# zhen8838/K210_Yolo_framework

Measured on AMD Instinct MI355X. Metric: images/sec end-to-end, yolo_mobilev1-0.75 320x240 b32 (`value_from_host`: SURVEY 8(d) end to end - u8 frames in pinned host memory -> H2D -> normalise -> backbone + heads -> decode -> NMS -> detections in host memory; `value`: the same step with the frames already resident in HBM, which is what the , higher is better.
Workload: dtype f16x2 (compensated fp16 MFMA operands: x = hi + lo, fp32 accumulate)

## Files before the change

### k210_yolo_framework_amd/csrc/yk_exact.hip

```cpp
#include <algorithm>
#include <math.h>
#include <string>
#include <vector>

#include "yk_conv.h"
#include "yk_plan_graph.h"

namespace {

typedef __attribute__((address_space(3))) void *lds_ptr_t;
typedef uint32_t u32x4 __attribute__((ext_vector_type(4)));
typedef uint32_t u32x2 __attribute__((ext_vector_type(2)));
#define X_OOB 0x40000000u
#ifdef YK_DEV
#define X_DBG(a, bit) (((a).dbg & (bit)) != 0)
#else
#define X_DBG(a, bit) false
#endif

extern __shared__ __attribute__((aligned(16))) unsigned char xsm[];

__device__ __forceinline__ float x_actf(float v, float slope, float cap) { return __builtin_amdgcn_fmed3f(v, v * slope, cap); }
__device__ __forceinline__ uint32_t x_div(uint32_t n, yk_fastdiv d) { return (__umulhi(n, d.mul) + n) >> d.shift; }

// ... 825 lines not shown
    x_amax_lds(&smax, 0, mx);
    __syncthreads();
    if (tid == 0 && smax) x_amax_global(a.amax_out + (size_t)b * XS, smax);
}

enum { XK_STEM = 1, XK_CONV, XK_DW, XK_POOL, XK_ADD, XK_U8MAX, XK_BLOCK, XK_PERSIST, XK_HEADS, XK_FIN };
enum { XC_64x64 = 0, XC_64x128, XC_128x64, XC_128x128, XC_NUM };
struct xc_info {
    int bm, bn, threads;
    const char *name;
};
const xc_info g_xc[XC_NUM] = {{64, 64, 256, "64x64"}, {64, 128, 256, "64x128"}, {128, 64, 256, "128x64"}, {128, 128, 512, "128x128"}};

struct xtens : yk_gtens {
    uint8_t *d = nullptr;
    bool f32 = false;
    float *d32 = nullptr;
};
struct xlaunch {
    int kind = 0;
    xg_args c;
    xdw_args d;
    xstem_args s;
    xpool_args p;
    xadd_args ad;
    xb_args b;
    int tm = 0, tn = 0;
    int Ho = 0, Wo = 0;
    int cfg = 0, ns = 2;
    unsigned lds = 0;
    int in_tid = -1, out_tid = -1;
    unsigned ring_lds = 0;
    xp_args pa;
    xh_args ha;
    unsigned h_lds = 0;
    xf_args f;
    int fin_bn = 0;
    int p_cw = 0;
    std::string name;
    double flops = 0, bytes = 0;
};

template <int BM, int BN, int WM, int WN, int NS>
int x_launch_g(const xg_args &g, hipStream_t st) {
    typedef xg_cfg<BM, BN, WM, WN> C;
    constexpr unsigned lds = (unsigned)C::lds(NS), rlds = (unsigned)(C::CT + C::SMALL);
    dim3 grid((unsigned)((g.M + BM - 1) / BM), (unsigned)((g.N + BN - 1) / BN), (unsigned)g.splitk);
    yk_launch_lds(g.splitk > 1 ? xg_kernel<BM, BN, WM, WN, NS, true> : xg_kernel<BM, BN, WM, WN, NS, false>, grid, dim3(C::NT), lds, st, g);
    if (g.splitk > 1) yk_launch_lds(xg_reduce_kernel<BM, BN, WM, WN>, dim3(grid.x, grid.y), dim3(C::NT), rlds, st, g);
    return YK_OK;
}
template <int BM, int BN, int WM, int WN>
int x_launch_g_ns(const xg_args &g, int ns, hipStream_t st) {
    if (ns <= 2) return x_launch_g<BM, BN, WM, WN, 2>(g, st);
    if (ns == 3) return x_launch_g<BM, BN, WM, WN, 3>(g, st);
    return x_launch_g<BM, BN, WM, WN, 4>(g, st);
}
int x_launch_conv(int cfg, int ns, const xg_args &g, hipStream_t st) {
    switch (cfg) {
    case XC_64x64: return x_launch_g_ns<64, 64, 2, 2>(g, ns, st);
    case XC_64x128: return x_launch_g_ns<64, 128, 2, 2>(g, ns, st);
    case XC_128x64: return x_launch_g_ns<128, 64, 2, 2>(g, ns, st);
    case XC_128x128: return x_launch_g_ns<128, 128, 2, 4>(g, std::min(ns, 3), st);
    }
    yk_set_error("f16x2: bad tile configuration %d", cfg);
    return YK_ERR_ARG;
}

template <int BM, int BN, int NW>
int x_launch_fin_bn(const xf_args &f, int ns, hipStream_t st) {
    typedef xf_cfg<BM, BN, NW> C;
    const dim3 grid((unsigned)((f.c.M + BM - 1) / BM), 1u, (unsigned)f.c.splitk);
    if (ns < 3) yk_launch_lds(xf_kernel<BM, BN, 2, NW>, grid, dim3(C::NT), C::lds(2), st, f);
    else yk_launch_lds(xf_kernel<BM, BN, 3, NW>, grid, dim3(C::NT), C::lds(3), st, f);
    return YK_OK;
}
int x_launch_fin(int bn, int ns, const xf_args &f, hipStream_t st) {
    if (bn == 128) return x_launch_fin_bn<64, 128, 4>(f, ns, st);
    if (bn == 192) return x_launch_fin_bn<64, 192, 4>(f, ns, st);
    yk_set_error("f16x2: no fused head kernel for a 64 x %d tile on 4 waves", bn);
    return YK_ERR_ARG;
}

template <int TM, int TN, int SG, bool F32IN = false>
int x_launch_b2(const xb_args &g, int batch, unsigned lds, hipStream_t st) {
    if constexpr (SG > 0 && !F32IN)
        if (g.in_f32) return x_launch_b2<TM, TN, SG, true>(g, batch, lds, st);
    dim3 grid((unsigned)(batch * g.tiles_x * g.tiles_y), (unsigned)((g.N + 64 * TN - 1) / (64 * TN)));
    yk_launch_lds(xb_kernel<TM, TN, SG, F32IN>, grid, dim3(256), lds, st, g);
    return YK_OK;
}
template <int TM, int TN>
int x_launch_b(const xb_args &g, int batch, unsigned lds, hipStream_t st) {
    if constexpr (TN == 1) {
        if (g.stem && g.GL == 2) return x_launch_b2<TM, TN, 2>(g, batch, lds, st);
        if (g.stem && g.GL == 3) return x_launch_b2<TM, TN, 3>(g, batch, lds, st);
        if (g.stem && g.GL == 4) return x_launch_b2<TM, TN, 4>(g, batch, lds, st);
    }
    if (g.stem) {
        yk_set_error("f16x2: stem fusion needs an N tile of 64 and 16, 24 or 32 stem filters");
        return YK_ERR_UNSUPPORTED;
    }
    return x_launch_b2<TM, TN, 0>(g, batch, lds, st);
}
const int g_xb_tm[] = {2, 3, 4, 5, 8}, g_xb_tn[] = {1, 2, 3, 6};
bool xb_has(int tm, int tn) {
    if (tm * tn > 24) return false;
    bool a = false, b = false;
    for (int v : g_xb_tm) a |= v == tm;
    for (int v : g_xb_tn) b |= v == tn;
    return a && b;
}
int x_launch_block(int tm, int tn, const xb_args &g, int batch, unsigned lds, hipStream_t st) {
#define XB_CASE(M, N) \
    if (tm == M && tn == N) return x_launch_b<M, N>(g, batch, lds, st);
    XB_CASE(2, 1) XB_CASE(2, 2) XB_CASE(2, 3) XB_CASE(2, 6)
    XB_CASE(3, 1) XB_CASE(3, 2) XB_CASE(3, 3) XB_CASE(3, 6)
    XB_CASE(4, 1) XB_CASE(4, 2) XB_CASE(4, 3) XB_CASE(4, 6)
    XB_CASE(5, 1) XB_CASE(5, 2) XB_CASE(5, 3)
    XB_CASE(8, 1) XB_CASE(8, 2) XB_CASE(8, 3)
#undef XB_CASE
    yk_set_error("f16x2: no fused block kernel <%d,%d>", tm, tn);
    return YK_ERR_ARG;
}
int xb_bt_bytes(int tn, int N) { return std::min(64 * tn, (N + 15) / 16 * 16) * 128; }
unsigned xb_lds(int tm, int tn, int n16p, int db, int N, bool wt = false, bool staged = true) {
    const int bm = 16 * tm, bn = 64 * tn;
    const int ipp = (tn >= 3 && tm >= 2) ? (tm + 1) / 2 : tm;
    const int ring = (db ? 2 : 1) * (n16p * 32 + 2048 + (wt ? xb_bt_bytes(tn, N) : 0)) + bm * 128, ct = staged ? ipp * 16 * (bn * 4 + 16) : 0;
    return (unsigned)(std::max(ring, ct) + 64);
}
bool xb_geometry(xb_args &g, int *tm_out, int *tn_out, unsigned *lds_out, int max_batch, int ordinal) {
    const int s = g.stride;
    double best = -1.0;
    const bool mine = !yk_dev_env("YK_XB_LAYER") || atoi(yk_dev_env("YK_XB_LAYER")) == ordinal;
    const int force_tm = mine && yk_dev_env("YK_XB_TM") ? atoi(yk_dev_env("YK_XB_TM")) : 0, force_tn = mine && yk_dev_env("YK_XB_TN") ? atoi(yk_dev_env("YK_XB_TN")) : 0;
    const int force_tw = mine && yk_dev_env("YK_XB_TW") ? atoi(yk_dev_env("YK_XB_TW")) : 0;
    const int force_db = mine && yk_dev_env("YK_XB_DB") ? atoi(yk_dev_env("YK_XB_DB")) : -1;
    const bool forced = force_tm || force_tn || force_tw || force_db >= 0;
    const bool wide = g.N > 192 && g.nk > 6;
    const int tn_want = (wide && yk_dev_env("YK_XB_TNL")) ? atoi(yk_dev_env("YK_XB_TNL")) : (wide ? 6 : std::min(3, (g.N + 63) / 64));
    (void)max_batch;
    for (int tm : g_xb_tm)
        for (int tn : g_xb_tn) {
            if (!xb_has(tm, tn) || (force_tm && tm != force_tm) || (force_tn && tn != force_tn)) continue;
            if (!force_tn && tn != tn_want) continue;
            const int tm_long = yk_dev_env("YK_XB_TML") ? atoi(yk_dev_env("YK_XB_TML")) : 4;
            if (!force_tm && tm > (tn_want == 1 ? 8 : (g.nk > 6 ? tm_long : 4))) continue;
            const int bm = 16 * tm;
            for (int TW = 1; TW <= std::min(g.Wo, bm); ++TW) {
                if (force_tw && TW != force_tw) continue;
                const int TH = std::min(g.Ho, bm / TW);
                if (TH * TW <= 16 * (tm - 1)) continue;
                const int PH = (TH - 1) * s + 3, PW = (TW - 1) * s + 3;
                const int n16 = PH * PW * 4, n16p = (n16 + 63) & ~63;
                if (n16p > 1536) continue;
                for (int db = 0; db <= 1; ++db) {
                    if (force_db >= 0 ? db != force_db : db != 0) continue;
                    const unsigned lds = xb_lds(tm, tn, n16p, db, g.N);
                    if (lds > 160 * 1024 || (!forced && xb_lds(tm, tn, n16p, db, g.N, !wide) > 53 * 1024 + 512)) continue;
                    const long tiles = (long)((g.Ho + TH - 1) / TH) * ((g.Wo + TW - 1) / TW);
                    const double cover = (double)g.Ho * g.Wo / ((double)tiles * bm);
                    const double halo = (double)TH * TW * s * s / ((double)PH * PW);
                    const double score = bm * cover * (0.5 + 0.5 * halo) * (TW >= TH ? 1.0 : 0.999) * ((TW & 3) ? 0.98 : 1.0);
                    if (score > best) {
                        best = score;
                        *tm_out = tm; *tn_out = tn; *lds_out = lds;
                        g.TH = TH; g.TW = TW; g.PH = PH; g.PW = PW; g.n16 = n16; g.n16p = n16p; g.db = db;
                        g.lds_bytes = (int)lds;
                        g.prepass = (s == 1 && yk_dev_env("YK_XB_PREPASS")) ? 1 : 0;
                        g.tiles_x = (g.Wo + TW - 1) / TW;
                        g.tiles_y = (g.Ho + TH - 1) / TH;
                    }
                }
            }
        }
    if (best < 0) return false;
    g.fd_tpi = yk_make_fastdiv((uint32_t)(g.tiles_x * g.tiles_y));
    g.fd_tx = yk_make_fastdiv((uint32_t)g.tiles_x);
    g.fd_tw = yk_make_fastdiv((uint32_t)g.TW);
    g.fd_pw = yk_make_fastdiv((uint32_t)g.PW);
    g.fd_nk = yk_make_fastdiv((uint32_t)std::max(1, g.nk));
    g.GL = 4;
    return true;
}

}

struct yk_xplan {
    int max_batch = 0, in_h = 0, in_w = 0;
    std::vector<xtens> T;
    std::vector<xlaunch> L;
    yk_dev_mem mem;
    std::vector<int> outputs;
    unsigned *d_imgmax = nullptr;
    uint32_t *d_amax = nullptr;
    size_t zero_words = 0;
    uint32_t *d_err = nullptr;
    uint32_t *h_err = nullptr;
    int *d_eexp = nullptr;
    long long *d_dbg = nullptr;
    int dbg_launch = -1;
    int cluster_wt = 0;
};

void yk_xplan_destroy(yk_xplan *p) {
    if (!p) return;
    p->mem.free_all();
    if (p->h_err) (void)hipHostFree(p->h_err);
    delete p;
}


static int x_build_persist(yk_xplan *p, int max_batch) {
    constexpr int CW = 8;
    const unsigned ring_cap = XP_NS * 8 * 6 * 1024;
    auto pw_ok = [&](const xlaunch &l) {
        const xg_args &g = l.c;
        return l.kind == XK_CONV && g.ks == 1 && g.stride == 1 && !g.s1.p && !g.up0 && !g.res.p && g.splitk == 1 && g.out && l.in_tid >= 0 &&
               (g.N % (16 * CW)) == 0 && (g.s0.G % CW) == 0 && (g.s0.G % 4) == 0;
    };
    auto dw_ok = [&](const xlaunch &l) { return l.kind == XK_DW && (l.d.in.G % CW) == 0 && (l.d.in.G % 4) == 0; };
    auto y_fits = [&](int H, int W, int Gs) { return (unsigned)(2 * (H + 2) * (W + 2) * Gs * 16) <= ring_cap; };
    int best0 = -1, best1 = -1;
    const int n = (int)p->L.size();
    for (int i = 0; i < n; ++i) {
        if (!dw_ok(p->L[i])) continue;
        int k = i, blocks = 0;
        while (k + 1 < n && dw_ok(p->L[k]) && pw_ok(p->L[k + 1]) && p->L[k + 1].in_tid == p->L[k].out_tid && p->T[p->L[k].out_tid].uses == 1) {
            const xdw_args &d = p->L[k].d;
            const xg_args &g = p->L[k + 1].c;
            const int nrb = (d.Ho * d.Wo + 15) / 16, ncb = g.N / 16 / CW, nT = 2 * (nrb + ncb);
            bool ok = nT <= 48 && y_fits(d.in.H, d.in.W, d.in.G / CW) && y_fits(d.Ho, d.Wo, g.N / 8 / CW) && d.in.H * d.in.W <= 1024;
            bool tile = false;
            for (int wr = 8; wr >= 1 && !tile; wr >>= 1) tile = (nrb + wr - 1) / wr <= 3 && (ncb + 8 / wr - 1) / (8 / wr) <= 3;
            if (!ok || !tile) break;
            ++blocks;
            k += 2;
            if (!(k < n && dw_ok(p->L[k]) && p->L[k].in_tid == p->L[k - 1].out_tid)) break;
        }
        if (blocks >= 2 && blocks * 2 > best1 - best0 + 1) {
            best0 = i;
            best1 = i + 2 * blocks - 1;
        }
        if (blocks) i = i + 2 * blocks - 1;
    }
    if (best0 < 0) return YK_OK;
    std::vector<xp_phase> ph;
    std::vector<std::pair<uint32_t, const xlaunch *>> wcopy;
    uint32_t arena = 0, dmax = 0;
    double flops = 0, bytes = 0;
    int nbar = 0, dbuf = 0;
    auto zero_phase = [] {
        xp_phase q;
        memset(&q, 0, sizeof(q));
        return q;
    };
    for (int k = best0; k <= best1; k += 2) {
        const xlaunch &ld = p->L[k], &lp = p->L[k + 1];
        const xdw_args &d = ld.d;
        const xg_args &g = lp.c;
        flops += ld.flops + lp.flops;
        bytes += ld.bytes + lp.bytes;
        const int Gs_in = d.in.G / CW, Gs_out = g.N / 8 / CW;
        if (k == best0) {
            xp_phase q = zero_phase();
// ... 475 lines not shown
```

### k210_yolo_framework_amd/csrc/yk_xblock.h

```cpp
#pragma once

struct xb_args {
    xview in, res;
    int B, Ho, Wo, N;
    int stride, pad_t, pad_l;
    const float *par;
    int nk;
    float dw_slope, dw_cap, dw_gain, dw_off;
    const uint8_t *w;
    uint32_t w_bytes;
    int nslab;
    const float *scale, *bias;
    float slope, cap, gain, off;
    uint8_t *out;
    int outG;
    int *eexp_out;
    uint32_t *amax_out;
    int TH, TW, PH, PW, tiles_x, tiles_y, n16, n16p;
    int db;
    int prepass;
    int src_f32, dst_f32;
    int lds_bytes;
    yk_fastdiv fd_tpi, fd_tx, fd_tw, fd_pw, fd_nk;
    int stem;
    const void *frames;
    const unsigned *img_max;
    int in_f32, fH, fW;
    int st_stride, st_pad_t, st_pad_l, st_cout;
    const yk_half *st_wf;
    const float *st_scale, *st_bias;
    float st_slope, st_cap, st_bound;
    int st_e;
    yk_fastdiv fd_wrow;
    yk_fastdiv fd_dpr;
    int GL;
    int dbg;
    long long *stamps;
};

template <int TM, int TN>
struct xb_cfg {
    static constexpr int BM = 16 * TM, BN = 64 * TN;
    static constexpr int PARB = 2048;
    static constexpr int CPITCH = BN * 4 + 16;
    static constexpr int IPP = (TN >= 3 && TM >= 2) ? (TM + 1) / 2 : TM;
    static constexpr int stage(int n16p) { return n16p * 32 + PARB; }
    static constexpr int lds(int n16p, int db) {
        const int r = (db ? 2 : 1) * stage(n16p) + BM * 128, ct = IPP * 16 * CPITCH;
        return (r > ct ? r : ct) + 64;
    }
};

template <bool U8, int GL>
__device__ __forceinline__ void xb_stem_patch(const xb_args &a, const void *winp, int WC, int pitch, float inv, int iy0, int ix0, unsigned char *HI, unsigned char *LO) {
    const int lane = threadIdx.x & 63, wid = threadIdx.x >> 6, fr = lane & 15, fq = lane >> 4;
    half8 wfh[2], wfl[2];
    float scv[2][4], bsv[2][4];
    const float sdown = x_pow2(-a.st_e), sfac = U8 ? sdown / inv : sdown, cap = a.st_cap * sdown;
#pragma unroll
    for (int nf = 0; nf < 2; ++nf) {
        wfh[nf] = *reinterpret_cast<const half8 *>(a.st_wf + ((size_t)(nf * 2 + 0) * 64 + lane) * 8);
        wfl[nf] = *reinterpret_cast<const half8 *>(a.st_wf + ((size_t)(nf * 2 + 1) * 64 + lane) * 8);
        const float4 sc = *reinterpret_cast<const float4 *>(a.st_scale + nf * 16 + fq * 4);
        const float4 bs = *reinterpret_cast<const float4 *>(a.st_bias + nf * 16 + fq * 4);
        scv[nf][0] = sc.x * sfac, scv[nf][1] = sc.y * sfac, scv[nf][2] = sc.z * sfac, scv[nf][3] = sc.w * sfac;
        bsv[nf][0] = bs.x * sdown, bsv[nf][1] = bs.y * sdown, bsv[nf][2] = bs.z * sdown, bsv[nf][3] = bs.w * sdown;
    }
    const int st = a.st_stride, npos = a.PH * a.PW, nblk = (npos + 15) >> 4, rowf = WC * 3;
    for (int blk = wid; blk < nblk; blk += 4) {
        const int pos = blk * 16 + fr, pc = min(pos, npos - 1);
        const int r = (int)x_div((uint32_t)pc, a.fd_pw), c = pc - r * a.PW;
        const bool valid = pos < npos;
        const bool inside = valid && (unsigned)(iy0 + r) < (unsigned)a.in.H && (unsigned)(ix0 + c) < (unsigned)a.in.W;
        half8 xh, xl;
        if constexpr (U8) {
            const unsigned char *wb = reinterpret_cast<const unsigned char *>(winp);
            const int off = (r * st) * pitch + c * st * 3;
            uint32_t d0, d1 = 0u;
            if (fq < 3) {
                const int o = off + fq * pitch, sh = o & 3;
                const uint32_t *q = reinterpret_cast<const uint32_t *>(wb + (o & ~3));
                const uint32_t w0 = q[0], w1 = q[1], w2 = q[2];
                d0 = __builtin_amdgcn_alignbyte(w1, w0, sh);
                d1 = __builtin_amdgcn_alignbyte(w2, w1, sh);
            } else {
                d0 = (uint32_t)wb[off + 8] | ((uint32_t)wb[off + pitch + 8] << 8) | ((uint32_t)wb[off + 2 * pitch + 8] << 16);
            }
#pragma unroll
            for (int j = 0; j < 4; ++j) {
                xh[j] = (yk_half)(float)((d0 >> (8 * j)) & 255u);
                xh[4 + j] = (yk_half)(float)((d1 >> (8 * j)) & 255u);
            }
        } else {
            const float *base = reinterpret_cast<const float *>(winp) + ((r * st) * WC + c * st) * 3;
            float x[8];
            if (fq < 3) {
#pragma unroll
                for (int j = 0; j < 8; ++j) x[j] = base[fq * rowf + j];
            } else {
                x[0] = base[8];
                x[1] = base[rowf + 8];
                x[2] = base[2 * rowf + 8];
#pragma unroll
                for (int j = 3; j < 8; ++j) x[j] = 0.f;
            }
            x_split8(x, xh, xl);
        }
        floatx4 acc[2];
#pragma unroll
        for (int nf = 0; nf < 2; ++nf) acc[nf] = __builtin_amdgcn_mfma_f32_16x16x32_f16(wfl[nf], xh, floatx4{0.f, 0.f, 0.f, 0.f}, 0, 0, 0);
        if constexpr (!U8) {
#pragma unroll
            for (int nf = 0; nf < 2; ++nf) acc[nf] = __builtin_amdgcn_mfma_f32_16x16x32_f16(wfh[nf], xl, acc[nf], 0, 0, 0);
        }
#pragma unroll
        for (int nf = 0; nf < 2; ++nf) acc[nf] = __builtin_amdgcn_mfma_f32_16x16x32_f16(wfh[nf], xh, acc[nf], 0, 0, 0);
#pragma unroll
        for (int nf = 0; nf < 2; ++nf) {
            float v[4];
#pragma unroll
            for (int k = 0; k < 4; ++k) {
                const float u = __builtin_fmaf(acc[nf][k], scv[nf][k], bsv[nf][k]);
                v[k] = inside ? x_actf(u, a.st_slope, cap) : 0.f;
            }
            const int n = nf * 16 + fq * 4;
            if (valid && (n >> 3) < GL) {
                const int at = (pos * GL + (n >> 3)) * 16;
                *reinterpret_cast<u32x4 *>(((n & 4) ? LO : HI) + at) = u32x4{__float_as_uint(v[0]), __float_as_uint(v[1]), __float_as_uint(v[2]), __float_as_uint(v[3])};
            }
        }
    }
}

template <int TM, int TN, int SG, bool F32IN = false>
__global__ void __launch_bounds__(256, (TM * TN > 8 ? 2 : 4)) xb_kernel(const xb_args a) {
    typedef xb_cfg<TM, TN> C;
    constexpr int BM = C::BM, BN = C::BN;
    constexpr bool STEM = SG > 0;
    constexpr int GL = STEM ? SG : 4;
    const int tid = threadIdx.x, lane = tid & 63, wid = tid >> 6;
    const int G = a.in.G, s = a.stride;
#ifdef YK_DEV
    const int XB_DB = a.db, XB_PREPASS = a.prepass;
#else
    constexpr int XB_DB = 0, XB_PREPASS = 0;
#endif
#ifdef YK_DEV
#define XB_STAMP(k) \
    if (a.stamps && tid == 0) a.stamps[((size_t)blockIdx.y * gridDim.x + blockIdx.x) * 16 + (k)] = (long long)wall_clock64();
#else
#define XB_STAMP(k)
#endif
    XB_STAMP(0)
    const int STG = a.n16p * 32 + C::PARB;
    unsigned char *A = xsm + (XB_DB ? 2 : 1) * STG;
    float *sf = reinterpret_cast<float *>(xsm + a.lds_bytes - 64);
    uint32_t *smax = reinterpret_cast<uint32_t *>(sf + 8);
    const int bid = x_xcd_tile(blockIdx.x, gridDim.x);
    const uint32_t b = x_div((uint32_t)bid, a.fd_tpi), tl = bid - b * (a.tiles_x * a.tiles_y);
    const uint32_t ty = x_div(tl, a.fd_tx), tx = tl - ty * a.tiles_x;
    const int oy0 = (int)ty * a.TH, ox0 = (int)tx * a.TW;
    const int iy0 = oy0 * s - a.pad_t, ix0 = ox0 * s - a.pad_l;
    const int n0 = blockIdx.y * BN;
    const int fr = lane & 15, fq = lane >> 4, nl4 = fq * 4;
    constexpr bool EARLY_SB = TN <= 1;
    float4 sc[TN], bs[TN];
    if constexpr (EARLY_SB) {
#pragma unroll
        for (int j = 0; j < TN; ++j) {
            const int n = n0 + (wid * TN + j) * 16 + nl4;
            sc[j] = *reinterpret_cast<const float4 *>(a.scale + n);
            bs[j] = *reinterpret_cast<const float4 *>(a.bias + n);
        }
    }
    const uint32_t img = (uint32_t)a.in.H * a.in.W * G * 32u;
    const __amdgpu_buffer_rsrc_t rsx = __builtin_amdgcn_make_buffer_rsrc((void *)(STEM ? (const uint8_t *)a.par : a.in.p + (size_t)b * img), 0, STEM ? 16u : img, 0x00020000);
    const __amdgpu_buffer_rsrc_t rsp = __builtin_amdgcn_make_buffer_rsrc((void *)a.par, 0, (uint32_t)(11 * G * 32), 0x00020000);
    const __amdgpu_buffer_rsrc_t rsw = __builtin_amdgcn_make_buffer_rsrc((void *)a.w, 0, a.w_bytes, 0x00020000);
    constexpr int PQ = 6;
    uint32_t poff[PQ];
#pragma unroll
    for (int i = 0; i < PQ; ++i) {
        poff[i] = X_OOB;
        if (!STEM && i * 256 < a.n16p) {
            const uint32_t q = (uint32_t)(i * 256 + tid);
            const uint32_t pos = q >> 2, g4 = q & 3;
            const uint32_t r = x_div(pos, a.fd_pw), c = pos - r * a.PW;
            const int iy = iy0 + (int)r, ix = ix0 + (int)c;
            const bool ok = (int)q < a.n16 && (unsigned)iy < (unsigned)a.in.H && (unsigned)ix < (unsigned)a.in.W;
            poff[i] = ok ? (uint32_t)(((iy * a.in.W + ix) * G + (int)g4) * 32) : X_OOB;
        }
    }
    const int g4l = tid & 3;
    const int rot = (a.nk == 1 || X_DBG(a, 32)) ? 0 : (int)(tl - x_div(tl, a.fd_nk) * (uint32_t)a.nk);
    auto kstep = [&](int i) {
        const int k = i + rot;
        return k >= a.nk ? k - a.nk : k;
    };
    const uint32_t wstep = (uint32_t)a.nslab * 2048u;
    auto dma_patch = [&](int it_) {
        const int ks = kstep(it_);
        unsigned char *HI = xsm + ((XB_DB & it_) & 1) * STG, *LO = HI + a.n16p * 16, *PARb = HI + a.n16p * 32;
        const bool gok = (ks * 4 + g4l) < G;
        const uint32_t koff = gok ? (uint32_t)ks * 128u : X_OOB;
#pragma unroll
        for (int i = 0; i < PQ; ++i)
            if (!STEM && i * 256 + wid * 64 < a.n16p) {
                const uint32_t oh = poff[i] + koff, ol = oh + 16u;
                __builtin_amdgcn_raw_ptr_buffer_load_lds(rsx, (lds_ptr_t)(HI + (i * 256 + wid * 64) * 16), 16, oh, 0, 0, 0);
                __builtin_amdgcn_raw_ptr_buffer_load_lds(rsx, (lds_ptr_t)(LO + (i * 256 + wid * 64) * 16), 16, ol, 0, 0, 0);
            }
        if (wid < 2) {
            const int idx = wid * 64 + lane, t = idx >> 3, pc = idx & 7;
            const int ch = ks * 32 + pc * 4;
            const uint32_t op = (idx < 88 && ch < G * 8) ? (uint32_t)((t * G * 8 + ch) * 4) : X_OOB;
            __builtin_amdgcn_raw_ptr_buffer_load_lds(rsp, (lds_ptr_t)(PARb + wid * 1024), 16, op, 0, 0, 0);
        }
    };
    if (!X_DBG(a, 1)) dma_patch(0);
    if constexpr (STEM) {
        const int st = a.st_stride, WR = (a.PH - 1) * st + 3, WC = (a.PW - 1) * st + 3;
        const int wy0 = iy0 * st - a.st_pad_t, wx0 = ix0 * st - a.st_pad_l;
        float *win = reinterpret_cast<float *>(A);
        float inv = 1.f;
        if (!F32IN) {
            unsigned mx = 0;
#pragma unroll
            for (int j = 0; j < 32; ++j) mx = max(mx, a.img_max[b * 32 + j]);
            inv = (float)mx;
        }
        const int rowf_ = WC * 3;
        if constexpr (F32IN) {
            constexpr int WQ = 16;
            const float *f = reinterpret_cast<const float *>(a.frames);
            const size_t fimg = (size_t)b * a.fH * a.fW * 3;
            float wv[WQ];
            bool wok[WQ];
#pragma unroll
            for (int q = 0; q < WQ; ++q) {
                const int i = q * 256 + tid;
                const int r = (int)x_div((uint32_t)i, a.fd_wrow), rem = i - r * rowf_, c = rem / 3, ch = rem - c * 3;
                const int fy = wy0 + r, fx = wx0 + c;
                wok[q] = i < WR * rowf_ && (unsigned)fy < (unsigned)a.fH && (unsigned)fx < (unsigned)a.fW;
                wv[q] = f[wok[q] ? fimg + ((size_t)fy * a.fW + fx) * 3 + ch : fimg];
            }
#pragma unroll
            for (int q = 0; q < WQ; ++q) {
                const int i = q * 256 + tid;
                if (i < WR * rowf_) win[i] = wok[q] ? wv[q] : 0.f;
            }
        } else {
            constexpr int DQ = 5;
            const int dpr = (rowf_ + 3) >> 2;
            const uint32_t fbytes = (uint32_t)a.B * a.fH * a.fW * 3u;
            const __amdgpu_buffer_rsrc_t rsf = __builtin_amdgcn_make_buffer_rsrc((void *)a.frames, 0, fbytes, 0x00020000);
            const int rowb = a.fW * 3;
            u32x2 d2[DQ];
            int sh[DQ];
            uint32_t msk[DQ];
#pragma unroll
            for (int q = 0; q < DQ; ++q) {
                const int i = q * 256 + tid, r = (int)x_div((uint32_t)i, a.fd_dpr), d = i - r * dpr;
                const int fy = wy0 + r;
                const bool ok = r < WR && (unsigned)fy < (unsigned)a.fH;
                const int col = wx0 * 3 + d * 4;
                const int off = ((int)b * a.fH + fy) * rowb + col;
                sh[q] = off >= 0 ? (off & 3) * 8 : off * 8;
                d2[q] = __builtin_bit_cast(u32x2, __builtin_amdgcn_raw_buffer_load_b64(rsf, ok ? (uint32_t)(max(off, 0) & ~3) : X_OOB, 0, 0));
                const int lo = max(0, -col), hi = min(4, rowb - col);
                msk[q] = (ok && hi > lo) ? ((0xffffffffu << (8 * lo)) & (0xffffffffu >> (8 * (4 - hi)))) : 0u;
            }
#pragma unroll
            for (int q = 0; q < DQ; ++q) {
                const int i = q * 256 + tid;
                const unsigned long long v = ((unsigned long long)d2[q][1] << 32) | d2[q][0];
                const uint32_t dv = sh[q] >= 0 ? (uint32_t)(v >> sh[q]) : (uint32_t)(v << (-sh[q]));
                if (i < WR * dpr) reinterpret_cast<uint32_t *>(A)[i] = dv & msk[q];
            }
            if (tid < 2) reinterpret_cast<uint32_t *>(A)[WR * dpr + tid] = 0u;
        }
        XB_STAMP(11)
        __syncthreads();
        XB_STAMP(12)
        unsigned char *HI = xsm, *LO = xsm + a.n16p * 16;
        if constexpr (F32IN) xb_stem_patch<false, GL>(a, A, WC, 0, 1.f, iy0, ix0, HI, LO);
        else xb_stem_patch<true, GL>(a, A, WC, ((WC * 3 + 3) >> 2) * 4, inv, iy0, ix0, HI, LO);
    }
    XB_STAMP(1)
    if (wid == 0) {
        const float amax_in = STEM ? a.st_bound : x_amax_wave(a.in.amax, (int)b);
        const float bmid = fminf(a.dw_cap, a.dw_gain * amax_in + a.dw_off);
        float bout = fminf(a.cap, a.gain * bmid + a.off);
        float rup = 0.f;
        if (a.res.p) {
            bout += x_amax_wave(a.res.amax, (int)b);
            rup = x_pow2(a.res.eexp[b]);
        }
        const int em = x_exp_of(__float_as_uint(bmid)), eo = a.dst_f32 ? 0 : x_exp_of(__float_as_uint(bout));
        if (lane == 0) {
            sf[0] = x_pow2(STEM ? a.st_e : a.in.eexp[b]);
            sf[1] = x_pow2(-em);
            sf[2] = x_pow2(em);
            sf[3] = x_pow2(-eo);
            sf[4] = rup;
            smax[0] = 0u;
            a.eexp_out[b] = eo;
        }
    }
    XB_STAMP(2)
    floatx4 acc[TM][TN];
#pragma unroll
    for (int i = 0; i < TM; ++i)
#pragma unroll
        for (int j = 0; j < TN; ++j) acc[i][j] = floatx4{0.f, 0.f, 0.f, 0.f};
    const bool wave_live = n0 + wid * TN * 16 < a.N;
    const int foff = fr * 64 + ((fq ^ ((fr >> 1) & 3)) * 16);
    const int afoff = fr * (GL * 16) + (GL == 4 ? (fq ^ ((fr >> 1) & 3)) : (fq < GL ? fq : 0)) * 16;
    const int nk = X_DBG(a, 1) ? 0 : a.nk;
    for (int ks = 0; ks < nk; ++ks) {
        asm volatile("s_waitcnt vmcnt(0) lgkmcnt(0)" ::: "memory");
        __builtin_amdgcn_s_barrier();
        asm volatile("" ::: "memory");
        if (ks == 0) { XB_STAMP(3) }
        if (ks == 1) { XB_STAMP(13) }
        half8 wh[TN], wl[TN];
        if (wave_live && !X_DBG(a, 16)) {
            const uint32_t ws = (uint32_t)(n0 >> 4) * 2048u + (uint32_t)kstep(ks) * wstep + (uint32_t)(wid * TN) * 2048u + (uint32_t)foff;
#pragma unroll
            for (int j = 0; j < TN; ++j) {
                wh[j] = __builtin_bit_cast(half8, __builtin_amdgcn_raw_buffer_load_b128(rsw, ws + (uint32_t)j * 2048u, 0, 0));
                wl[j] = __builtin_bit_cast(half8, __builtin_amdgcn_raw_buffer_load_b128(rsw, ws + (uint32_t)j * 2048u + 1024u, 0, 0));
            }
        }
        if (XB_DB && ks + 1 < nk) dma_patch(ks + 1);
        const unsigned char *HI = xsm + ((XB_DB & ks) & 1) * STG, *LO = HI + a.n16p * 16;
        const unsigned char *PARB_ = HI + a.n16p * 32;
        const float up = sf[0], dmid = sf[1];
        const bool f32patch = STEM || XB_PREPASS || a.src_f32;
        if (!STEM && XB_PREPASS && !a.src_f32) {
            for (int e = tid; e < a.n16p; e += 256) {
                const u32x4 h = *reinterpret_cast<const u32x4 *>(HI + e * 16), l = *reinterpret_cast<const u32x4 *>(LO + e * 16);
                u32x4 x0, x1;
                x0[0] = __float_as_uint(x_mix_sum_lo(h[0], l[0])); x0[1] = __float_as_uint(x_mix_sum_hi(h[0], l[0]));
                x0[2] = __float_as_uint(x_mix_sum_lo(h[1], l[1])); x0[3] = __float_as_uint(x_mix_sum_hi(h[1], l[1]));
                x1[0] = __float_as_uint(x_mix_sum_lo(h[2], l[2])); x1[1] = __float_as_uint(x_mix_sum_hi(h[2], l[2]));
                x1[2] = __float_as_uint(x_mix_sum_lo(h[3], l[3])); x1[3] = __float_as_uint(x_mix_sum_hi(h[3], l[3]));
                *reinterpret_cast<u32x4 *>(const_cast<unsigned char *>(HI) + e * 16) = x0;
                *reinterpret_cast<u32x4 *>(const_cast<unsigned char *>(LO) + e * 16) = x1;
            }
            asm volatile("s_waitcnt lgkmcnt(0)" ::: "memory");
            __builtin_amdgcn_s_barrier();
            asm volatile("" ::: "memory");
        }
        if (!X_DBG(a, 2))
            for (int it = tid; it < BM * GL; it += 256) {
                int p, q;
                if constexpr (GL != 4) {
                    p = (int)((uint32_t)it / (uint32_t)GL);
                    q = it - p * GL;
                } else {
                    p = it >> 2;
                    q = it & 3;
                }
                const int py = (int)x_div((uint32_t)p, a.fd_tw), px = p - py * a.TW;
                const bool live = py < a.TH && oy0 + py < a.Ho && ox0 + px < a.Wo;
                half8 hi = {0, 0, 0, 0, 0, 0, 0, 0}, lo = hi;
                if (live) {
                    const int base = ((py * s) * a.PW + px * s) * GL + q;
                    float2v d2[4] = {{0.f, 0.f}, {0.f, 0.f}, {0.f, 0.f}, {0.f, 0.f}};
#pragma unroll
                    for (int t = 0; t < 9; ++t) {
#if defined(YK_KO) && (YK_KO & 2)
                        const int at = (base + ((t / 3) * a.PW) * GL) * 16;
#else
                        const int at = (base + ((t / 3) * a.PW + (t % 3)) * GL) * 16;
#endif
                        const u32x4 h = *reinterpret_cast<const u32x4 *>(HI + at), l = *reinterpret_cast<const u32x4 *>(LO + at);
#if defined(YK_KO) && (YK_KO & 1)
                        const u32x4 w0 = {0x3f000000u, 0x3e800000u, 0x3f000000u, 0x3e800000u}, w1 = w0;
#else
                        const u32x4 w0 = *reinterpret_cast<const u32x4 *>(PARB_ + (t * 32 + q * 8) * 4), w1 = *reinterpret_cast<const u32x4 *>(PARB_ + (t * 32 + q * 8 + 4) * 4);
#endif
                        const float2v w2[4] = {{__uint_as_float(w0[0]), __uint_as_float(w0[1])}, {__uint_as_float(w0[2]), __uint_as_float(w0[3])},
                                               {__uint_as_float(w1[0]), __uint_as_float(w1[1])}, {__uint_as_float(w1[2]), __uint_as_float(w1[3])}};
                        if (f32patch) {
                            d2[0] = __builtin_elementwise_fma(float2v{__uint_as_float(h[0]), __uint_as_float(h[1])}, w2[0], d2[0]);
                            d2[1] = __builtin_elementwise_fma(float2v{__uint_as_float(h[2]), __uint_as_float(h[3])}, w2[1], d2[1]);
                            d2[2] = __builtin_elementwise_fma(float2v{__uint_as_float(l[0]), __uint_as_float(l[1])}, w2[2], d2[2]);
                            d2[3] = __builtin_elementwise_fma(float2v{__uint_as_float(l[2]), __uint_as_float(l[3])}, w2[3], d2[3]);
                        } else {
#pragma unroll
                            for (int j = 0; j < 4; ++j) {
                                const float2v x2 = {x_mix_sum_lo(h[j], l[j]), x_mix_sum_hi(h[j], l[j])};
                                d2[j] = __builtin_elementwise_fma(x2, w2[j], d2[j]);
                            }
                        }
                    }
                    const float d[8] = {d2[0].x, d2[0].y, d2[1].x, d2[1].y, d2[2].x, d2[2].y, d2[3].x, d2[3].y};
                    const u32x4 s0_ = *reinterpret_cast<const u32x4 *>(PARB_ + (9 * 32 + q * 8) * 4), s1_ = *reinterpret_cast<const u32x4 *>(PARB_ + (9 * 32 + q * 8 + 4) * 4);
                    const u32x4 b0_ = *reinterpret_cast<const u32x4 *>(PARB_ + (10 * 32 + q * 8) * 4), b1_ = *reinterpret_cast<const u32x4 *>(PARB_ + (10 * 32 + q * 8 + 4) * 4);
                    const float scd[8] = {__uint_as_float(s0_[0]), __uint_as_float(s0_[1]), __uint_as_float(s0_[2]), __uint_as_float(s0_[3]),
                                          __uint_as_float(s1_[0]), __uint_as_float(s1_[1]), __uint_as_float(s1_[2]), __uint_as_float(s1_[3])};
                    const float bsd[8] = {__uint_as_float(b0_[0]), __uint_as_float(b0_[1]), __uint_as_float(b0_[2]), __uint_as_float(b0_[3]),
                                          __uint_as_float(b1_[0]), __uint_as_float(b1_[1]), __uint_as_float(b1_[2]), __uint_as_float(b1_[3])};
                    float vd[8];
#pragma unroll
                    for (int j = 0; j < 8; ++j) vd[j] = x_actf(__builtin_fmaf(d[j] * up, scd[j], bsd[j]), a.dw_slope, a.dw_cap) * dmid;
                    x_split8(vd, hi, lo);
                }
                const int r = p & 15;
                unsigned char *dst = A + (p >> 4) * (GL * 512) + r * (GL * 16) + ((q ^ (GL == 4 ? (r >> 1) & 3 : 0)) * 16);
                *reinterpret_cast<half8 *>(dst) = hi;
                *reinterpret_cast<half8 *>(dst + GL * 256) = lo;
            }
        if (ks == 0) { XB_STAMP(4) }
        if (ks == 1) { XB_STAMP(14) }
        asm volatile("s_waitcnt lgkmcnt(0)" ::: "memory");
        __builtin_amdgcn_s_barrier();
        asm volatile("" ::: "memory");
        if (ks == 0) { XB_STAMP(5) }
        if (ks == 1) { XB_STAMP(15) }
        if (!XB_DB && ks + 1 < nk) dma_patch(ks + 1);
        if (wave_live && !X_DBG(a, 16)) {
            half8 xh[TM], xl[TM];
#pragma unroll
            for (int i = 0; i < TM; ++i) {
                xh[i] = *reinterpret_cast<const half8 *>(A + i * (GL * 512) + afoff);
                xl[i] = *reinterpret_cast<const half8 *>(A + i * (GL * 512) + GL * 256 + afoff);
            }
#pragma unroll
            for (int i = 0; i < TM; ++i)
#pragma unroll
                for (int j = 0; j < TN; ++j)
                    acc[i][j] = __builtin_amdgcn_mfma_f32_16x16x32_f16(wl[j], xh[i], STEM ? floatx4{0.f, 0.f, 0.f, 0.f} : acc[i][j], 0, 0, 0);
#pragma unroll
            for (int i = 0; i < TM; ++i)
#pragma unroll
                for (int j = 0; j < TN; ++j) acc[i][j] = __builtin_amdgcn_mfma_f32_16x16x32_f16(wh[j], xl[i], acc[i][j], 0, 0, 0);
#pragma unroll
            for (int i = 0; i < TM; ++i)
#pragma unroll
                for (int j = 0; j < TN; ++j) acc[i][j] = __builtin_amdgcn_mfma_f32_16x16x32_f16(wh[j], xh[i], acc[i][j], 0, 0, 0);
        }
    }
    XB_STAMP(6)
    asm volatile("s_waitcnt vmcnt(0) lgkmcnt(0)" ::: "memory");
    __builtin_amdgcn_s_barrier();
    asm volatile("" ::: "memory");
    XB_STAMP(7)
    if (X_DBG(a, 4)) return;
    unsigned char *Cs = xsm;
    const float umid = sf[2], dout = sf[3], rup = sf[4];
    float rmax = 0.f;
    constexpr int VPR = BN / 4, IPP = C::IPP;
    if constexpr (!EARLY_SB) {
#pragma unroll
        for (int j = 0; j < TN; ++j) {
            const int n = n0 + (wid * TN + j) * 16 + nl4;
            sc[j] = *reinterpret_cast<const float4 *>(a.scale + n);
            bs[j] = *reinterpret_cast<const float4 *>(a.bias + n);
        }
    }
    float4 scu[TN];
#pragma unroll
    for (int j = 0; j < TN; ++j) scu[j] = float4{sc[j].x * umid, sc[j].y * umid, sc[j].z * umid, sc[j].w * umid};
    if (a.dst_f32 && !a.res.p) {
        if (wave_live) {
            const uint32_t oimg = (uint32_t)a.Ho * a.Wo * a.outG * 32u;
            const __amdgpu_buffer_rsrc_t rso = __builtin_amdgcn_make_buffer_rsrc((void *)(a.out + (size_t)b * oimg), 0, oimg, 0x00020000);
#pragma unroll
            for (int i = 0; i < TM; ++i) {
                const int p = i * 16 + fr;
                const int py = (int)x_div((uint32_t)p, a.fd_tw), px = p - py * a.TW;
                const int oy = oy0 + py, ox = ox0 + px;
                const bool mok = py < a.TH && oy < a.Ho && ox < a.Wo;
                const uint32_t po = (uint32_t)((oy * a.Wo + ox) * a.outG) * 32u;
#pragma unroll
                for (int j = 0; j < TN; ++j) {
                    const int n = n0 + (wid * TN + j) * 16 + nl4;
                    float v[4];
                    v[0] = x_actf(__builtin_fmaf(acc[i][j][0], scu[j].x, bs[j].x), a.slope, a.cap);
                    v[1] = x_actf(__builtin_fmaf(acc[i][j][1], scu[j].y, bs[j].y), a.slope, a.cap);
                    v[2] = x_actf(__builtin_fmaf(acc[i][j][2], scu[j].z, bs[j].z), a.slope, a.cap);
                    v[3] = x_actf(__builtin_fmaf(acc[i][j][3], scu[j].w, bs[j].w), a.slope, a.cap);
                    if (mok && (n >> 3) < a.outG) {
#pragma unroll
                        for (int k = 0; k < 4; ++k) rmax = fmaxf(rmax, fabsf(v[k]));
                        __builtin_amdgcn_raw_buffer_store_b128(u32x4{__float_as_uint(v[0]), __float_as_uint(v[1]), __float_as_uint(v[2]), __float_as_uint(v[3])}, rso,
                                                               po + (uint32_t)((n >> 3) * 32 + ((n >> 2) & 1) * 16), 0, 0);
                    }
                }
            }
        }
        x_amax_lds(smax, 0, rmax);
        __syncthreads();
        if (tid == 0 && smax[0]) x_amax_global(a.amax_out + (size_t)b * XS, smax[0]);
        XB_STAMP(9)
        XB_STAMP(10)
        return;
    }
    const uint32_t simg = (uint32_t)a.Ho * a.Wo * a.outG * 32u, rimg = (uint32_t)a.Ho * a.Wo * a.res.G * 32u;
    const __amdgpu_buffer_rsrc_t rss = __builtin_amdgcn_make_buffer_rsrc((void *)(a.out + (size_t)b * simg), 0, simg, 0x00020000);
    const __amdgpu_buffer_rsrc_t rsr = __builtin_amdgcn_make_buffer_rsrc((void *)(a.res.p ? a.res.p + (size_t)b * rimg : a.out), 0, a.res.p ? rimg : 0u, 0x00020000);
#pragma unroll
    for (int i0 = 0; i0 < TM; i0 += IPP) {
        if (i0 > 0) __syncthreads();
#pragma unroll
        for (int i = i0; i < i0 + IPP && i < TM; ++i) {
            if (!wave_live && wid != 0) break;
            const int p = i * 16 + fr;
            const int py = (int)x_div((uint32_t)p, a.fd_tw), px = p - py * a.TW;
            const int oy = oy0 + py, ox = ox0 + px;
            const bool mok = py < a.TH && oy < a.Ho && ox < a.Wo;
            const int m = oy * a.Wo + ox;
            if (wid == 0 && fq == 0) *reinterpret_cast<int *>(Cs + (p - i0 * 16) * C::CPITCH + BN * 4) = mok ? m : -1;
#pragma unroll
            for (int j = 0; j < TN; ++j) {
                const int nl = (wid * TN + j) * 16 + nl4, n = n0 + nl;
                float v[4];
                v[0] = x_actf(__builtin_fmaf(acc[i][j][0], scu[j].x, bs[j].x), a.slope, a.cap);
                v[1] = x_actf(__builtin_fmaf(acc[i][j][1], scu[j].y, bs[j].y), a.slope, a.cap);
                v[2] = x_actf(__builtin_fmaf(acc[i][j][2], scu[j].z, bs[j].z), a.slope, a.cap);
                v[3] = x_actf(__builtin_fmaf(acc[i][j][3], scu[j].w, bs[j].w), a.slope, a.cap);
                if (a.res.p && mok && (n >> 3) < a.res.G) {
                    const uint32_t q = (uint32_t)((m * a.res.G + (n >> 3)) * 32 + (n & 7) * 2), q2 = q + 16u;
                    const half4 rh = __builtin_bit_cast(half4, __builtin_amdgcn_raw_buffer_load_b64(rsr, q, 0, 0));
                    const half4 rl = __builtin_bit_cast(half4, __builtin_amdgcn_raw_buffer_load_b64(rsr, q2, 0, 0));
#pragma unroll
                    for (int k = 0; k < 4; ++k) v[k] += ((float)rh[k] + (float)rl[k]) * rup;
                }
#pragma unroll
                for (int k = 0; k < 4; ++k)
                    if (mok) rmax = fmaxf(rmax, fabsf(v[k]));
                if (a.dst_f32) {
                    *reinterpret_cast<u32x4 *>(Cs + (p - i0 * 16) * C::CPITCH + (nl >> 3) * 32 + ((nl >> 2) & 1) * 16) =
                        u32x4{__float_as_uint(v[0]), __float_as_uint(v[1]), __float_as_uint(v[2]), __float_as_uint(v[3])};
                } else {
                    half4 hi, lo;
                    float vd[4];
#pragma unroll
                    for (int k = 0; k < 4; ++k) vd[k] = v[k] * dout;
                    x_split4(vd, hi, lo);
                    unsigned char *d = Cs + (p - i0 * 16) * C::CPITCH + (nl >> 3) * 32 + (nl & 7) * 2;
                    *reinterpret_cast<half4 *>(d) = hi;
                    *reinterpret_cast<half4 *>(d + 16) = lo;
                }
            }
        }
        if (i0 == 0) { XB_STAMP(8) }
        const bool last = i0 + IPP >= TM;
        if (last) x_amax_lds(smax, 0, rmax);
        __syncthreads();
        if (last && tid == 0 && smax[0]) x_amax_global(a.amax_out + (size_t)b * XS, smax[0]);
        const int rows = (TM - i0 < IPP ? TM - i0 : IPP) * 16;
        for (int v = tid; v < rows * VPR; v += 256) {
            const int pr = v / VPR, cv = v - pr * VPR;
            const int m = *reinterpret_cast<const int *>(Cs + pr * C::CPITCH + BN * 4), g = (n0 >> 3) + (cv >> 1);
            const uint32_t so = (m >= 0 && g < a.outG) ? (uint32_t)((m * a.outG + g) * 32 + (cv & 1) * 16) : X_OOB;
            __builtin_amdgcn_raw_buffer_store_b128(*reinterpret_cast<const u32x4 *>(Cs + pr * C::CPITCH + cv * 16), rss, so, 0, 0);
        }
    }
    XB_STAMP(9)
    XB_STAMP(10)
#undef XB_STAMP
}
```

Baseline: 80170.

## Run wide fused dw+pw block kernels on 8 waves splitting N slabs

Adds an 8-wave (512-thread) variant of the fused depthwise+pointwise block kernel for TN=6 tiles. Each wave now owns half as many 16-column N slabs, so accumulators and weight registers per wave shrink. The depthwise patch prologue is split into half-groups so all 8 waves share that work. The aim is more latency hiding and less register pressure per wave on wide layers. The cost is extra barrier participants, a 2-blocks-per-CU bound, and a second code path for the depthwise stage.

```diff
diff --git a/k210_yolo_framework_amd/csrc/yk_exact.hip b/k210_yolo_framework_amd/csrc/yk_exact.hip
--- a/k210_yolo_framework_amd/csrc/yk_exact.hip
+++ b/k210_yolo_framework_amd/csrc/yk_exact.hip
@@ -931,12 +931,12 @@
     return YK_ERR_ARG;
 }
 
-template <int TM, int TN, int SG, bool F32IN = false>
+template <int TM, int TN, int SG, bool F32IN = false, int NW = 4>
 int x_launch_b2(const xb_args &g, int batch, unsigned lds, hipStream_t st) {
     if constexpr (SG > 0 && !F32IN)
         if (g.in_f32) return x_launch_b2<TM, TN, SG, true>(g, batch, lds, st);
     dim3 grid((unsigned)(batch * g.tiles_x * g.tiles_y), (unsigned)((g.N + 64 * TN - 1) / (64 * TN)));
-    yk_launch_lds(xb_kernel<TM, TN, SG, F32IN>, grid, dim3(256), lds, st, g);
+    yk_launch_lds(xb_kernel<TM, TN, SG, F32IN, NW>, grid, dim3(NW * 64), lds, st, g);
     return YK_OK;
 }
 template <int TM, int TN>
@@ -949,6 +949,13 @@
     if (g.stem) {
         yk_set_error("f16x2: stem fusion needs an N tile of 64 and 16, 24 or 32 stem filters");
         return YK_ERR_UNSUPPORTED;
+    }
+    if constexpr (TN == 6) {
+        if (g.waves == 8) return x_launch_b2<TM, TN, 0, false, 8>(g, batch, lds, st);
+    }
+    if (g.waves != 4) {
+        yk_set_error("f16x2: no fused block kernel <%d,%d> on %d waves", TM, TN, g.waves);
+        return YK_ERR_ARG;
     }
     return x_launch_b2<TM, TN, 0>(g, batch, lds, st);
 }
@@ -1031,6 +1038,7 @@
     g.fd_pw = yk_make_fastdiv((uint32_t)g.PW);
     g.fd_nk = yk_make_fastdiv((uint32_t)std::max(1, g.nk));
     g.GL = 4;
+    g.waves = (wide && *tn_out == 6 && !(yk_dev_env("YK_XB_WAVES") && atoi(yk_dev_env("YK_XB_WAVES")) == 4)) ? 8 : 4;
     return true;
 }
 
diff --git a/k210_yolo_framework_amd/csrc/yk_xblock.h b/k210_yolo_framework_amd/csrc/yk_xblock.h
--- a/k210_yolo_framework_amd/csrc/yk_xblock.h
+++ b/k210_yolo_framework_amd/csrc/yk_xblock.h
@@ -34,6 +34,7 @@
     yk_fastdiv fd_wrow;
     yk_fastdiv fd_dpr;
     int GL;
+    int waves;
     int dbg;
     long long *stamps;
 };
@@ -132,11 +133,14 @@
     }
 }
 
-template <int TM, int TN, int SG, bool F32IN = false>
-__global__ void __launch_bounds__(256, (TM * TN > 8 ? 2 : 4)) xb_kernel(const xb_args a) {
+template <int TM, int TN, int SG, bool F32IN = false, int NW = 4>
+__global__ void __launch_bounds__(NW * 64, (NW == 8 || TM * TN > 8 ? 2 : 4)) xb_kernel(const xb_args a) {
     typedef xb_cfg<TM, TN> C;
     constexpr int BM = C::BM, BN = C::BN;
     constexpr bool STEM = SG > 0;
+    constexpr int NT = NW * 64;
+    constexpr int TNW = TN * 4 / NW;
+    static_assert(NW == 4 || (NW == 8 && !STEM && (TN & 1) == 0), "8 waves: stored-tensor blocks with an even number of slabs per 4 waves");
     constexpr int GL = STEM ? SG : 4;
     const int tid = threadIdx.x, lane = tid & 63, wid = tid >> 6;
     const int G = a.in.G, s = a.stride;
@@ -164,11 +168,11 @@
     const int n0 = blockIdx.y * BN;
     const int fr = lane & 15, fq = lane >> 4, nl4 = fq * 4;
     constexpr bool EARLY_SB = TN <= 1;
-    float4 sc[TN], bs[TN];
+    float4 sc[TNW], bs[TNW];
     if constexpr (EARLY_SB) {
 #pragma unroll
-        for (int j = 0; j < TN; ++j) {
-            const int n = n0 + (wid * TN + j) * 16 + nl4;
+        for (int j = 0; j < TNW; ++j) {
+            const int n = n0 + (wid * TNW + j) * 16 + nl4;
             sc[j] = *reinterpret_cast<const float4 *>(a.scale + n);
             bs[j] = *reinterpret_cast<const float4 *>(a.bias + n);
         }
@@ -177,13 +181,13 @@
     const __amdgpu_buffer_rsrc_t rsx = __builtin_amdgcn_make_buffer_rsrc((void *)(STEM ? (const uint8_t *)a.par : a.in.p + (size_t)b * img), 0, STEM ? 16u : img, 0x00020000);
     const __amdgpu_buffer_rsrc_t rsp = __builtin_amdgcn_make_buffer_rsrc((void *)a.par, 0, (uint32_t)(11 * G * 32), 0x00020000);
     const __amdgpu_buffer_rsrc_t rsw = __builtin_amdgcn_make_buffer_rsrc((void *)a.w, 0, a.w_bytes, 0x00020000);
-    constexpr int PQ = 6;
+    constexpr int PQ = 6 * 4 / NW;
     uint32_t poff[PQ];
 #pragma unroll
     for (int i = 0; i < PQ; ++i) {
         poff[i] = X_OOB;
-        if (!STEM && i * 256 < a.n16p) {
-            const uint32_t q = (uint32_t)(i * 256 + tid);
+        if (!STEM && i * NT < a.n16p) {
+            const uint32_t q = (uint32_t)(i * NT + tid);
             const uint32_t pos = q >> 2, g4 = q & 3;
             const uint32_t r = x_div(pos, a.fd_pw), c = pos - r * a.PW;
             const int iy = iy0 + (int)r, ix = ix0 + (int)c;
@@ -205,10 +209,10 @@
         const uint32_t koff = gok ? (uint32_t)ks * 128u : X_OOB;
 #pragma unroll
         for (int i = 0; i < PQ; ++i)
-            if (!STEM && i * 256 + wid * 64 < a.n16p) {
+            if (!STEM && i * NT + wid * 64 < a.n16p) {
                 const uint32_t oh = poff[i] + koff, ol = oh + 16u;
-                __builtin_amdgcn_raw_ptr_buffer_load_lds(rsx, (lds_ptr_t)(HI + (i * 256 + wid * 64) * 16), 16, oh, 0, 0, 0);
-                __builtin_amdgcn_raw_ptr_buffer_load_lds(rsx, (lds_ptr_t)(LO + (i * 256 + wid * 64) * 16), 16, ol, 0, 0, 0);
+                __builtin_amdgcn_raw_ptr_buffer_load_lds(rsx, (lds_ptr_t)(HI + (i * NT + wid * 64) * 16), 16, oh, 0, 0, 0);
+                __builtin_amdgcn_raw_ptr_buffer_load_lds(rsx, (lds_ptr_t)(LO + (i * NT + wid * 64) * 16), 16, ol, 0, 0, 0);
             }
         if (wid < 2) {
             const int idx = wid * 64 + lane, t = idx >> 3, pc = idx & 7;
@@ -308,12 +312,12 @@
         }
     }
     XB_STAMP(2)
-    floatx4 acc[TM][TN];
+    floatx4 acc[TM][TNW];
 #pragma unroll
     for (int i = 0; i < TM; ++i)
 #pragma unroll
-        for (int j = 0; j < TN; ++j) acc[i][j] = floatx4{0.f, 0.f, 0.f, 0.f};
-    const bool wave_live = n0 + wid * TN * 16 < a.N;
+        for (int j = 0; j < TNW; ++j) acc[i][j] = floatx4{0.f, 0.f, 0.f, 0.f};
+    const bool wave_live = n0 + wid * TNW * 16 < a.N;
     const int foff = fr * 64 + ((fq ^ ((fr >> 1) & 3)) * 16);
     const int afoff = fr * (GL * 16) + (GL == 4 ? (fq ^ ((fr >> 1) & 3)) : (fq < GL ? fq : 0)) * 16;
     const int nk = X_DBG(a, 1) ? 0 : a.nk;
@@ -323,11 +327,11 @@
         asm volatile("" ::: "memory");
         if (ks == 0) { XB_STAMP(3) }
         if (ks == 1) { XB_STAMP(13) }
-        half8 wh[TN], wl[TN];
+        half8 wh[TNW], wl[TNW];
         if (wave_live && !X_DBG(a, 16)) {
-            const uint32_t ws = (uint32_t)(n0 >> 4) * 2048u + (uint32_t)kstep(ks) * wstep + (uint32_t)(wid * TN) * 2048u + (uint32_t)foff;
-#pragma unroll
-            for (int j = 0; j < TN; ++j) {
+            const uint32_t ws = (uint32_t)(n0 >> 4) * 2048u + (uint32_t)kstep(ks) * wstep + (uint32_t)(wid * TNW) * 2048u + (uint32_t)foff;
+#pragma unroll
+            for (int j = 0; j < TNW; ++j) {
                 wh[j] = __builtin_bit_cast(half8, __builtin_amdgcn_raw_buffer_load_b128(rsw, ws + (uint32_t)j * 2048u, 0, 0));
                 wl[j] = __builtin_bit_cast(half8, __builtin_amdgcn_raw_buffer_load_b128(rsw, ws + (uint32_t)j * 2048u + 1024u, 0, 0));
             }
@@ -338,7 +342,7 @@
         const float up = sf[0], dmid = sf[1];
         const bool f32patch = STEM || XB_PREPASS || a.src_f32;
         if (!STEM && XB_PREPASS && !a.src_f32) {
-            for (int e = tid; e < a.n16p; e += 256) {
+            for (int e = tid; e < a.n16p; e += NT) {
                 const u32x4 h = *reinterpret_cast<const u32x4 *>(HI + e * 16), l = *reinterpret_cast<const u32x4 *>(LO + e * 16);
                 u32x4 x0, x1;
                 x0[0] = __float_as_uint(x_mix_sum_lo(h[0], l[0])); x0[1] = __float_as_uint(x_mix_sum_hi(h[0], l[0]));
@@ -352,7 +356,7 @@
             __builtin_amdgcn_s_barrier();
             asm volatile("" ::: "memory");
         }
-        if (!X_DBG(a, 2))
+        if (NW == 4 && !X_DBG(a, 2))
             for (int it = tid; it < BM * GL; it += 256) {
                 int p, q;
                 if constexpr (GL != 4) {
@@ -413,6 +417,49 @@
                 *reinterpret_cast<half8 *>(dst) = hi;
                 *reinterpret_cast<half8 *>(dst + GL * 256) = lo;
             }
+        if constexpr (NW == 8) {
+            if (!X_DBG(a, 2))
+                for (int it = tid; it < BM * GL * 2; it += NT) {
+                    const int hf = it >= BM * GL ? 1 : 0, ih = it - hf * (BM * GL);
+                    const int p = ih >> 2, q = ih & 3;
+                    const int py = (int)x_div((uint32_t)p, a.fd_tw), px = p - py * a.TW;
+                    const bool live = py < a.TH && oy0 + py < a.Ho && ox0 + px < a.Wo;
+                    half4 hi = {0, 0, 0, 0}, lo = hi;
+                    if (live) {
+                        const int base = ((py * s) * a.PW + px * s) * GL + q;
+                        const unsigned char *PW_ = PARB_ + (q * 8 + hf * 4) * 4;
+                        float2v d2[2] = {{0.f, 0.f}, {0.f, 0.f}};
+#pragma unroll
+                        for (int t = 0; t < 9; ++t) {
+                            const int at = (base + ((t / 3) * a.PW + (t % 3)) * GL) * 16;
+                            const u32x4 w0 = *reinterpret_cast<const u32x4 *>(PW_ + t * 128);
+                            const float2v w2[2] = {{__uint_as_float(w0[0]), __uint_as_float(w0[1])}, {__uint_as_float(w0[2]), __uint_as_float(w0[3])}};
+                            if (f32patch) {
+                                const u32x4 x = *reinterpret_cast<const u32x4 *>((hf ? LO : HI) + at);
+                                d2[0] = __builtin_elementwise_fma(float2v{__uint_as_float(x[0]), __uint_as_float(x[1])}, w2[0], d2[0]);
+                                d2[1] = __builtin_elementwise_fma(float2v{__uint_as_float(x[2]), __uint_as_float(x[3])}, w2[1], d2[1]);
+                            } else {
+                                const u32x2 h = *reinterpret_cast<const u32x2 *>(HI + at + hf * 8), l = *reinterpret_cast<const u32x2 *>(LO + at + hf * 8);
+#pragma unroll
+                                for (int j = 0; j < 2; ++j) {
+                                    const float2v x2 = {x_mix_sum_lo(h[j], l[j]), x_mix_sum_hi(h[j], l[j])};
+                                    d2[j] = __builtin_elementwise_fma(x2, w2[j], d2[j]);
+                                }
+                            }
+                        }
+                        const float d[4] = {d2[0].x, d2[0].y, d2[1].x, d2[1].y};
+                        const u32x4 s0_ = *reinterpret_cast<const u32x4 *>(PW_ + 9 * 128), b0_ = *reinterpret_cast<const u32x4 *>(PW_ + 10 * 128);
+                        float vd[4];
+#pragma unroll
+                        for (int j = 0; j < 4; ++j) vd[j] = x_actf(__builtin_fmaf(d[j] * up, __uint_as_float(s0_[j]), __uint_as_float(b0_[j])), a.dw_slope, a.dw_cap) * dmid;
+                        x_split4(vd, hi, lo);
+                    }
+                    const int r = p & 15;
+                    unsigned char *dst = A + (p >> 4) * (GL * 512) + r * (GL * 16) + ((q ^ ((r >> 1) & 3)) * 16) + hf * 8;
+                    *reinterpret_cast<half4 *>(dst) = hi;
+                    *reinterpret_cast<half4 *>(dst + GL * 256) = lo;
+                }
+        }
         if (ks == 0) { XB_STAMP(4) }
         if (ks == 1) { XB_STAMP(14) }
         asm volatile("s_waitcnt lgkmcnt(0)" ::: "memory");
@@ -431,16 +478,16 @@
 #pragma unroll
             for (int i = 0; i < TM; ++i)
 #pragma unroll
-                for (int j = 0; j < TN; ++j)
+                for (int j = 0; j < TNW; ++j)
                     acc[i][j] = __builtin_amdgcn_mfma_f32_16x16x32_f16(wl[j], xh[i], STEM ? floatx4{0.f, 0.f, 0.f, 0.f} : acc[i][j], 0, 0, 0);
 #pragma unroll
             for (int i = 0; i < TM; ++i)
 #pragma unroll
-                for (int j = 0; j < TN; ++j) acc[i][j] = __builtin_amdgcn_mfma_f32_16x16x32_f16(wh[j], xl[i], acc[i][j], 0, 0, 0);
+                for (int j = 0; j < TNW; ++j) acc[i][j] = __builtin_amdgcn_mfma_f32_16x16x32_f16(wh[j], xl[i], acc[i][j], 0, 0, 0);
 #pragma unroll
             for (int i = 0; i < TM; ++i)
 #pragma unroll
-                for (int j = 0; j < TN; ++j) acc[i][j] = __builtin_amdgcn_mfma_f32_16x16x32_f16(wh[j], xh[i], acc[i][j], 0, 0, 0);
+                for (int j = 0; j < TNW; ++j) acc[i][j] = __builtin_amdgcn_mfma_f32_16x16x32_f16(wh[j], xh[i], acc[i][j], 0, 0, 0);
         }
     }
     XB_STAMP(6)
@@ -455,15 +502,15 @@
     constexpr int VPR = BN / 4, IPP = C::IPP;
     if constexpr (!EARLY_SB) {
 #pragma unroll
-        for (int j = 0; j < TN; ++j) {
-            const int n = n0 + (wid * TN + j) * 16 + nl4;
+        for (int j = 0; j < TNW; ++j) {
+            const int n = n0 + (wid * TNW + j) * 16 + nl4;
             sc[j] = *reinterpret_cast<const float4 *>(a.scale + n);
             bs[j] = *reinterpret_cast<const float4 *>(a.bias + n);
         }
     }
-    float4 scu[TN];
-#pragma unroll
-    for (int j = 0; j < TN; ++j) scu[j] = float4{sc[j].x * umid, sc[j].y * umid, sc[j].z * umid, sc[j].w * umid};
+    float4 scu[TNW];
+#pragma unroll
+    for (int j = 0; j < TNW; ++j) scu[j] = float4{sc[j].x * umid, sc[j].y * umid, sc[j].z * umid, sc[j].w * umid};
     if (a.dst_f32 && !a.res.p) {
         if (wave_live) {
             const uint32_t oimg = (uint32_t)a.Ho * a.Wo * a.outG * 32u;
@@ -476,8 +523,8 @@
                 const bool mok = py < a.TH && oy < a.Ho && ox < a.Wo;
                 const uint32_t po = (uint32_t)((oy * a.Wo + ox) * a.outG) * 32u;
 #pragma unroll
-                for (int j = 0; j < TN; ++j) {
-                    const int n = n0 + (wid * TN + j) * 16 + nl4;
+                for (int j = 0; j < TNW; ++j) {
+                    const int n = n0 + (wid * TNW + j) * 16 + nl4;
                     float v[4];
                     v[0] = x_actf(__builtin_fmaf(acc[i][j][0], scu[j].x, bs[j].x), a.slope, a.cap);
                     v[1] = x_actf(__builtin_fmaf(acc[i][j][1], scu[j].y, bs[j].y), a.slope, a.cap);
@@ -515,8 +562,8 @@
             const int m = oy * a.Wo + ox;
             if (wid == 0 && fq == 0) *reinterpret_cast<int *>(Cs + (p - i0 * 16) * C::CPITCH + BN * 4) = mok ? m : -1;
 #pragma unroll
-            for (int j = 0; j < TN; ++j) {
-                const int nl = (wid * TN + j) * 16 + nl4, n = n0 + nl;
+            for (int j = 0; j < TNW; ++j) {
+                const int nl = (wid * TNW + j) * 16 + nl4, n = n0 + nl;
                 float v[4];
                 v[0] = x_actf(__builtin_fmaf(acc[i][j][0], scu[j].x, bs[j].x), a.slope, a.cap);
                 v[1] = x_actf(__builtin_fmaf(acc[i][j][1], scu[j].y, bs[j].y), a.slope, a.cap);
@@ -553,7 +600,7 @@
         __syncthreads();
         if (last && tid == 0 && smax[0]) x_amax_global(a.amax_out + (size_t)b * XS, smax[0]);
         const int rows = (TM - i0 < IPP ? TM - i0 : IPP) * 16;
-        for (int v = tid; v < rows * VPR; v += 256) {
+        for (int v = tid; v < rows * VPR; v += NT) {
             const int pr = v / VPR, cv = v - pr * VPR;
             const int m = *reinterpret_cast<const int *>(Cs + pr * C::CPITCH + BN * 4), g = (n0 >> 3) + (cv >> 1);
             const uint32_t so = (m >= 0 && g < a.outG) ? (uint32_t)((m * a.outG + g) * 32 + (cv & 1) * 16) : X_OOB;
```

New measurement: 81550, median of 6. 1.7% higher.
